# EricLBuehler/mistral.rs

Measured on AMD Instinct MI355X. Metric: decode_tokens_per_sec, higher is better.
Workload: dtype q4_k/q6_k weights x q8_k activations (int8 dot, f32 accumulate: the reference CPU path's arithmetic); 1 GPU; Llama-3-8B GGUF Q4_K_M, TP=1, 512 prefill / 1598 decode, batch 1, paged KV bf16 (block 32); parallelism=tp1

## Files before the change

### mistral.rs_amd/csrc/ext_dec.hip

```cpp
#include "dec_attn.cuh"
#include <stdio.h>
#include <stdlib.h>
#include <math.h>
#include <algorithm>
#include "../../include/mistralrs_paged_attn.h"

#include "dec_gemv.cuh"

#ifndef MRS_WAIT_VMCNT0
#define MRS_WAIT_VMCNT0() asm volatile("s_waitcnt vmcnt(0)" ::: "memory")
#endif

namespace mrs {
namespace dec {

__device__ __forceinline__ void st16(uint8_t *p, const uint8_t *b) { *(v4u *)p = *(const v4u *)b; }
__device__ __forceinline__ void k4_scale_min(const uint8_t *sc12, uint8_t *sc, uint8_t *mn) {
#pragma unroll
  for (int g = 0; g < 8; ++g) {
    if (g < 4) { sc[g] = sc12[g] & 63; mn[g] = sc12[g + 4] & 63; }
    else { sc[g] = (sc12[g + 4] & 15) | ((sc12[g - 4] >> 6) << 4); mn[g] = (sc12[g + 4] >> 4) | ((sc12[g] >> 6) << 4); }
  }
}
template <int TYPE>
__global__ void __launch_bounds__(256) repack_kernel(const uint8_t *__restrict__ src, uint8_t *__restrict__ dst, long long n, int K, long long nlanes) {
  const long long i = (long long)blockIdx.x * 256 + threadIdx.x;
  if (i >= nlanes) return;
  const Geo g = geo_for(K);
  const long long tile = i >> 6;
  const int L = (int)(i & 63), r = L >> 4, p = (L >> 2) & 3, c = L & 3, slot = L >> 2;
  const long long rg = tile / g.Cs;
  const int t = (int)(tile - rg * g.Cs);
  const long long row = rg * g.R + r;
  const int sb = p * g.Cs + t;
  const bool have = row < n && sb < g.S;
  uint8_t *tb = dst + (size_t)tile * tile_bytes(TYPE);
  alignas(16) uint8_t buf[16];
  if constexpr (TYPE == T_Q4_K || TYPE == T_Q5_K) {
    constexpr int TS = TYPE == T_Q4_K ? 144 : 176;
    constexpr unsigned HS = TYPE == T_Q4_K ? 2048u : 2560u, HD = TYPE == T_Q4_K ? 2304u : 2816u;
    const uint8_t *b = src + ((size_t)row * g.S + sb) * TS;
    const uint8_t *qs = b + (TYPE == T_Q5_K ? 48 : 16);
    for (int h = 0; h < 2; ++h) {
      for (int k = 0; k < 16; ++k) buf[k] = have ? (uint8_t)(qs[32 * c + 16 * h + k] ^ (TYPE == T_Q4_K ? 0x80 : 0x00)) : 0;
      st16(tb + (size_t)h * 1024 + (size_t)L * 16, buf);
    }
    if constexpr (TYPE == T_Q5_K) {
      const uint8_t *qh = b + 16;
      for (int h = 0; h < 2; ++h) {
        uint32_t wv = 0;
        if (have)
          for (int k = 0; k < 4; ++k)
            for (int jj = 0; jj < 4; ++jj) {
              const uint32_t v = qh[h * 16 + 4 * k + jj];
              wv |= ((v >> (2 * c)) & 1u) << (8 * jj + k);
              wv |= ((v >> (2 * c + 1)) & 1u) << (8 * jj + 4 + k);
            }
        *(uint32_t *)(tb + 2048 + (size_t)L * 8 + 4 * h) = wv;
      }
    }
    uint8_t sc[8], mn[8];
    if (have) k4_scale_min(b + 4, sc, mn);
    *(uint32_t *)(tb + HS + (size_t)L * 4) = have ? ((uint32_t)sc[2 * c] | ((uint32_t)sc[2 * c + 1] << 8) | ((uint32_t)mn[2 * c] << 16) | ((uint32_t)mn[2 * c + 1] << 24)) : 0u;
    if (c == 0) *(uint32_t *)(tb + HD + (size_t)slot * 4) = have ? ((uint32_t)b[0] | ((uint32_t)b[1] << 8) | ((uint32_t)b[2] << 16) | ((uint32_t)b[3] << 24)) : 0u;
  } else if constexpr (TYPE == T_Q6_K) {
    const uint8_t *b = src + ((size_t)row * g.S + sb) * 210;
    const uint8_t *ql = b, *qh = b + 128;
    auto lo4 = [&](int e) { const int hh = e / 128, pos = e % 32, qt = (e % 128) / 32, ii = hh * 64 + pos + (qt % 2) * 32; return qt < 2 ? (ql[ii] & 15) : (ql[ii] >> 4); };
    auto hi2 = [&](int e) { const int hh = e / 128, pos = e % 32, qt = (e % 128) / 32; return (qh[hh * 32 + pos] >> (qt * 2)) & 3; };
    for (int h = 0; h < 2; ++h) {
      for (int k = 0; k < 16; ++k) buf[k] = have ? (uint8_t)(lo4((4 * c + 2 * h) * 16 + k) | (lo4((4 * c + 2 * h + 1) * 16 + k) << 4)) : 0;
      st16(tb + (size_t)h * 1024 + (size_t)L * 16, buf);
    }
    for (int k = 0; k < 16; ++k)
      buf[k] = have ? (uint8_t)(hi2((4 * c) * 16 + k) | (hi2((4 * c + 1) * 16 + k) << 2) | (hi2((4 * c + 2) * 16 + k) << 4) | (hi2((4 * c + 3) * 16 + k) << 6)) : 0;
    st16(tb + 2048 + (size_t)L * 16, buf);
    *(uint32_t *)(tb + 3072 + (size_t)L * 4) = have ? ((uint32_t)b[192 + 4 * c] | ((uint32_t)b[193 + 4 * c] << 8) | ((uint32_t)b[194 + 4 * c] << 16) | ((uint32_t)b[195 + 4 * c] << 24)) : 0u;
    if (c == 0) *(uint16_t *)(tb + 3328 + (size_t)slot * 2) = have ? (uint16_t)(b[208] | (b[209] << 8)) : (uint16_t)0;
  } else {
    const uint8_t *b = src + ((size_t)row * (K / 32) + (size_t)sb * 8 + 2 * c) * 34;
    for (int pi = 0; pi < 4; ++pi) {
      for (int k = 0; k < 16; ++k) buf[k] = have ? b[(pi >> 1) * 34 + 2 + (pi & 1) * 16 + k] : 0;
      st16(tb + (size_t)pi * 1024 + (size_t)L * 16, buf);
    }
    *(uint32_t *)(tb + 4096 + (size_t)L * 4) = have ? ((uint32_t)b[0] | ((uint32_t)b[1] << 8) | ((uint32_t)b[34] << 16) | ((uint32_t)b[35] << 24)) : 0u;
  }
}

static bool make_mat(Mat &m, const void *planes, int type, long long n, long long k) {
  if (!planes || !dec_type(type) || n <= 0 || k <= 0 || k % 256) return false;
  const size_t tb = tensor_bytes(type, n, k);
  if (tb >= 0xF0000000ull) return false;
  m.base = (const uint8_t *)planes; m.bytes = (unsigned)tb; m.type = type; m.n = (int)n; m.k = (int)k;
  return true;
}


struct Attn2Args {
  AttnArgs t;
  unsigned *ticket;
  uint8_t *img;
};
template <int G>
__device__ __forceinline__ void attn2_merge(const Attn2Args &a, int kvh, int seq, int ns, int wave, int lane, int ncols) {
  constexpr int HD = 128, NP = (G + 1) / 2;
  const AttnArgs &t = a.t;
  if (wave >= NP) return;
  const int head0 = kvh * G, hsel = lane >> 5, head = head0 + 2 * wave + hsel;
  const bool live = 2 * wave + hsel < G;
  const size_t pA = ((size_t)seq * t.num_heads + head0 + 2 * wave) * t.max_splits;
  const size_t pB = ((size_t)seq * t.num_heads + head0 + min(2 * wave + 1, G - 1)) * t.max_splits;
  auto ldw = [&](const float *p) { return __hip_atomic_load(p, __ATOMIC_RELAXED, __HIP_MEMORY_SCOPE_AGENT); };
  const float mA = lane < ns ? ldw(t.part_m + pA + lane) : -FLT_MAX, lA = lane < ns ? ldw(t.part_l + pA + lane) : 0.f;
  const float mB = lane < ns ? ldw(t.part_m + pB + lane) : -FLT_MAX, lB = lane < ns ? ldw(t.part_l + pB + lane) : 0.f;
  const __amdgpu_buffer_rsrc_t ro = __builtin_amdgcn_make_buffer_rsrc((void *)(t.part_o + pA * HD), (short)0, (int)((pB - pA + ns) * HD * 4), 0x00020000);
  const unsigned off0 = (unsigned)(lane & 31) * 16u + (hsel ? (unsigned)((pB - pA) * HD * 4) : 0u);
  constexpr int MB = 16;
  constexpr int AUX = 16;
  v4u r[MB];
#pragma unroll
  for (int i = 0; i < MB; ++i) r[i] = __builtin_amdgcn_raw_buffer_load_b128(ro, off0 + (unsigned)i * 512u, 0, AUX);
  const float wA = fast_exp_ref(mA - dec2::wave_max_all(mA)), wB = fast_exp_ref(mB - dec2::wave_max_all(mB));
  float s_all = 0.f;
  float4 acc = make_float4(0.f, 0.f, 0.f, 0.f);
  auto step = [&](int j, v4u raw) {
    const float wAj = dec2::rlf(wA, j), wBj = dec2::rlf(wB, j), lAj = dec2::rlf(lA, j), lBj = dec2::rlf(lB, j);
    const float wj = hsel ? wBj : wAj, lj = hsel ? lBj : lAj;
    const float lw = lj * wj;
    s_all = s_all + lw;
    const float4 o = as_f4(raw);
    const float t0 = o.x * wj, t1 = o.y * wj, t2 = o.z * wj, t3 = o.w * wj;
    acc.x = acc.x + t0; acc.y = acc.y + t1; acc.z = acc.z + t2; acc.w = acc.w + t3;
  };
  for (int j0 = 0; j0 < ns; j0 += MB) {
    if (j0 > 0) {
#pragma unroll
      for (int i = 0; i < MB; ++i) r[i] = __builtin_amdgcn_raw_buffer_load_b128(ro, off0 + (unsigned)(j0 + i) * 512u, 0, AUX);
    }
#pragma unroll
    for (int i = 0; i < MB; ++i)
      if (j0 + i < ns) step(j0 + i, r[i]);
  }
  const float inv = 1.0f / s_all;
  const float4 v = make_float4(acc.x * inv, acc.y * inv, acc.z * inv, acc.w * inv);
  if (t.out && live) *(float4 *)(t.out + ((size_t)seq * t.num_heads + head) * HD + (lane & 31) * 4) = v;
  if (a.img) {
    const int K = t.num_heads * HD, sb = (head0 + 2 * wave) >> 1;
    quantize_sb(v, sb, seq, ACT_Q8K, (char *)a.img, K, ncols);
  }
}

template <int G, class CT>
__global__ void __launch_bounds__(64 * G) dec_attn2_kernel(const Attn2Args a) {
  constexpr int HD = 128;
  __shared__ __attribute__((aligned(16))) float q_s[G][HD + 32];
  __shared__ int last_s;
  const AttnArgs &t = a.t;
  const int tid = tid_opaque(), lane = tid & 63, wave = __builtin_amdgcn_readfirstlane(tid >> 6);
  const int kvh = blockIdx.x, seq = blockIdx.y;
  const int split = blockIdx.z, head0 = kvh * G;
  const unsigned blk_first = t.block_tables[(size_t)seq * t.max_blocks_per_seq + min(split * t.bpw, t.max_blocks_per_seq - 1)];
  const int nblk = ((int)t.context_lens[seq] + 31) / 32;
  const int ns = (nblk + t.bpw - 1) / t.bpw;
  if (split >= ns) return;
  {
    const int b0 = split * t.bpw, b1 = min(b0 + t.bpw, nblk);
    const int ctx_w = (int)t.context_lens[seq], lo_w = t.window > 0 && ctx_w > t.window ? ctx_w - t.window : 0;
    auto publish = [&](int, float o0, float o1, float m, float l) {
      const size_t pi = ((size_t)seq * t.num_heads + head0 + wave) * t.max_splits + split;
      __hip_atomic_store(t.part_o + pi * HD + lane, o0, __ATOMIC_RELAXED, __HIP_MEMORY_SCOPE_AGENT);
      __hip_atomic_store(t.part_o + pi * HD + lane + 64, o1, __ATOMIC_RELAXED, __HIP_MEMORY_SCOPE_AGENT);
      if (lane == 0) {
        __hip_atomic_store(t.part_m + pi, m, __ATOMIC_RELAXED, __HIP_MEMORY_SCOPE_AGENT);
        __hip_atomic_store(t.part_l + pi, l, __ATOMIC_RELAXED, __HIP_MEMORY_SCOPE_AGENT);
      }
    };
    if (b1 * 32 <= lo_w) {
      publish(0, 0.f, 0.f, -FLT_MAX, 0.f);
    } else {
      attn_split_core<1, CT>(t, kvh, head0 + wave, seq, b0, b1, q_s[wave], q_s[wave] + HD, publish, (int)blk_first);
    }
  }
  MRS_WAIT_VMCNT0();
  __syncthreads();
  unsigned *tk = a.ticket + (size_t)seq * t.num_kv_heads + kvh;
  constexpr int ticket_order = __ATOMIC_RELAXED;
  if (tid == 0) last_s = __hip_atomic_fetch_add(tk, 1u, ticket_order, __HIP_MEMORY_SCOPE_AGENT) == (unsigned)(ns - 1);
  __syncthreads();
  if (!last_s) return;
  if (tid == 0) __hip_atomic_store(tk, 0u, __ATOMIC_RELAXED, __HIP_MEMORY_SCOPE_AGENT);
  attn2_merge<G>(a, kvh, seq, ns, wave, lane, gridDim.y);
}


struct ActImgArgs {
  const float *x; int ldx; const float *norm_w; float eps; int K, mode;
  char *img;
  int gc0[8], gn[8];
};
__global__ void __launch_bounds__(NT) dec_act_image_kernel(const ActImgArgs a) {
  __shared__ float red[8];
  const int tid = tid_opaque(), wave = __builtin_amdgcn_readfirstlane(tid >> 6);
  const int c = (int)blockIdx.x;
  const float *x = a.x + (size_t)c * a.ldx;
  const ActRegs<1> pre = act_issue_all<1>(x, (unsigned)a.K * 4u, a.norm_w, a.K, wave);
  act_sumsq_all<1, 1>(red, pre, x, a.ldx, a.norm_w, a.K, wave);
  if (a.norm_w) __syncthreads();
  const int c0 = a.gc0[c], n = a.gn[c];
  act_quantize_all<1, 1>(a.img + act_bytes(a.K, c0), red, pre, x, a.ldx, a.norm_w, a.eps, a.K, a.mode, wave, c - c0, n);
}

static unsigned long long *g_tl_buf = nullptr;
template <int EPI> struct Launch {
  template <int NCOLS> static int go(GemvArgs a, hipStream_t s) {
    const Geo g = geo_for(a.K);
    constexpr int NCI = EPI == EPI_RESID2 ? 2 : NCOLS;
    a.tl = g_tl_buf;
    a.rgpu = EPI == EPI_QKV && g.R < 2 ? 2 : 1;
    const int upr = g.R * a.rgpu;
    int grid = 0;
    if (EPI == EPI_QKV) {
      double bytes[3]; double tot = 0; int want = 0;
      for (int i = 0; i < 3; ++i) {
        if (a.nrows[i] % upr) return -3;
        a.units[i] = a.nrows[i] / upr;
        bytes[i] = (double)a.units[i] * a.rgpu * g.TPC * (double)rec_bytes(a.m[i].type, g); tot += bytes[i]; want += a.units[i];
      }
      const int G = want < 256 ? want : 256;
      int wgs[3], used = 0;
      for (int i = 0; i < 3; ++i) { wgs[i] = std::max(1, std::min(a.units[i], (int)(G * bytes[i] / tot + 0.5))); used += wgs[i]; }
      while (used > G) { int big = 0; for (int i = 1; i < 3; ++i) if (wgs[i] > wgs[big]) big = i; if (wgs[big] <= 1) break; --wgs[big]; --used; }
      a.wg0[0] = 0; for (int i = 0; i < 3; ++i) a.wg0[i + 1] = a.wg0[i] + wgs[i];
      grid = a.wg0[3];
    } else {
      const int slots = a.slots > 1 ? a.slots : 1;
      if ((slots > 1 || a.expert_sel) && a.nrows[0] % upr) return -3;
      const int upe = (a.nrows[0] + upr - 1) / upr;
      a.units[0] = upe * slots;
      grid = a.units[0] < 256 ? a.units[0] : 256;
    }
    if (grid < 1) return -1;
    for (int i = 0; i < (EPI == EPI_QKV ? 3 : 1); ++i) {
      const int nwg = EPI == EPI_QKV ? a.wg0[i + 1] - a.wg0[i] : grid;
      a.ubase[i] = a.units[i] / nwg; a.urem[i] = a.units[i] % nwg;
    }
    a.upe = EPI == EPI_RESID2 ? a.units[0] : a.units[0] / (a.slots > 1 ? a.slots : 1);
    if (a.upe < 1) a.upe = 1;
    size_t lds = (act_bytes(a.K, NCI) + 15) & ~(size_t)15;
    if (lds > LDS_IMG_MAX) return -2;
    int tmask = 0;
    for (int i = 0; i < (EPI == EPI_QKV ? 3 : 1); ++i) tmask |= tmask_of(a.m[i].type);
    int total_units = 0;
    for (int i = 0; i < (EPI == EPI_QKV ? 3 : 1); ++i) total_units += a.units[i];
    static const int force_ring2 = [] { const char *e = getenv("MRS_DEC_RING2"); return e ? atoi(e) : -1; }();
    const bool ring2 = force_ring2 >= 0 ? force_ring2 != 0 : total_units >= 8 * grid;
    return gemv_launch<NCOLS>(EPI, tmask, ring2, grid, lds, a, s);
  }
  static GemvArgs shift_cols(GemvArgs a, int c0) {
    if (a.x) a.x += (size_t)c0 * a.ldx;
    if (a.out) a.out += (size_t)c0 * a.out_stride;
    if (a.qkv.q_out) a.qkv.q_out += (size_t)c0 * a.nrows[0];
    if (a.qkv.positions) a.qkv.positions += c0;
    if (a.qkv.slot_mapping) a.qkv.slot_mapping += c0;
    if (a.x_img) a.x_img = (const char *)a.x_img + act_bytes(a.K, c0);
    return a;
  }
  static int run(const GemvArgs &a, int b, hipStream_t s) {
    if (b > 1 && act_bytes(a.K, b) > LDS_IMG_MAX) {
      const int half = b / 2;
      const int rc = run(a, half, s);
      return rc ? rc : run(shift_cols(a, half), b - half, s);
    }
    switch (b) {
    case 1: return go<1>(a, s); case 2: return go<2>(a, s); case 3: return go<3>(a, s); case 4: return go<4>(a, s);
    case 5: return go<5>(a, s); case 6: return go<6>(a, s); case 7: return go<7>(a, s); case 8: return go<8>(a, s);
    default: return -1;
    }
  }
};

}
}

using namespace mrs;
using namespace mrs::dec;

struct mrs_dec_mat_c { const void *planes; int type; long long n, k; };

extern "C" void mrs_dec_timeline(void *buf, int) { g_tl_buf = (unsigned long long *)buf; }
extern "C" int mrs_dec_supported(int ggml_type) { return dec_type(ggml_type) ? 1 : 0; }
extern "C" size_t mrs_dec_repack_bytes(int type, long long n, long long k) {
  if (!dec_type(type) || k <= 0 || k % 256 || n <= 0) return 0;
  return tensor_bytes(type, n, k);
}
extern "C" int mrs_dec_repack(const void *gguf_blocks, int type, long long n, long long k, void *planes, void *stream) {
  if (!mrs_dec_repack_bytes(type, n, k) || !gguf_blocks || !planes) return -1;
  const Geo g = geo_for((int)k);
  const long long nslots = ((n + g.R - 1) / g.R) * g.TPC * 64;
  const dim3 grid((unsigned)((nslots + 255) / 256));
  hipStream_t s = (hipStream_t)stream;
  switch (type) {
  case T_Q4_K: hipLaunchKernelGGL(repack_kernel<T_Q4_K>, grid, dim3(256), 0, s, (const uint8_t *)gguf_blocks, (uint8_t *)planes, n, (int)k, nslots); break;
  case T_Q5_K: hipLaunchKernelGGL(repack_kernel<T_Q5_K>, grid, dim3(256), 0, s, (const uint8_t *)gguf_blocks, (uint8_t *)planes, n, (int)k, nslots); break;
  case T_Q6_K: hipLaunchKernelGGL(repack_kernel<T_Q6_K>, grid, dim3(256), 0, s, (const uint8_t *)gguf_blocks, (uint8_t *)planes, n, (int)k, nslots); break;
  default: hipLaunchKernelGGL(repack_kernel<T_Q8_0>, grid, dim3(256), 0, s, (const uint8_t *)gguf_blocks, (uint8_t *)planes, n, (int)k, nslots); break;
  }
  return 0;
}
static int dec_qkv_impl(const mrs_dec_mat_c *wq, const mrs_dec_mat_c *wk, const mrs_dec_mat_c *wv, const float *h, int ldh, const float *norm_w, float eps,
                        float *q_out, void *k_cache, void *v_cache, const int64_t *slot_mapping, const int32_t *positions, const float *cos_t,
                        const float *sin_t, int head_dim, int rot_pairs, int num_kv_heads, int block_size, int kv_dtype, int b, int neox, void *stream,
                        const void *x_img = nullptr) {
  GemvArgs a{};
  a.neox = neox;
  a.x_img = x_img;
  if (neox && rot_pairs * 2 != head_dim) return -1;
  if (!wq || !wk || !wv || !make_mat(a.m[0], wq->planes, wq->type, wq->n, wq->k) || !make_mat(a.m[1], wk->planes, wk->type, wk->n, wk->k) ||
      !make_mat(a.m[2], wv->planes, wv->type, wv->n, wv->k)) return -1;
  if (wq->k != wk->k || wq->k != wv->k) return -1;
  if (act_mode_for(wq->type) != act_mode_for(wk->type) || act_mode_for(wq->type) != act_mode_for(wv->type)) return -1;
  if (!qkv_epi_fill(a.qkv, q_out, k_cache, v_cache, slot_mapping, positions, cos_t, sin_t, head_dim, rot_pairs, num_kv_heads, block_size, kv_dtype, wq->n, wk->n, wv->n))
    return -1;
  a.nrows[0] = (int)wq->n; a.nrows[1] = (int)wk->n; a.nrows[2] = (int)wv->n; a.K = (int)wq->k;
  a.x = h; a.ldx = ldh; a.norm_w = norm_w; a.eps = eps;
  return Launch<EPI_QKV>::run(a, b, (hipStream_t)stream);
}
extern "C" int mrs_dec_qkv(const mrs_dec_mat_c *wq, const mrs_dec_mat_c *wk, const mrs_dec_mat_c *wv, const float *h, int ldh, const float *norm_w, float eps,
                           float *q_out, void *k_cache, void *v_cache, const int64_t *slot_mapping, const int32_t *positions, const float *cos_t,
                           const float *sin_t, int head_dim, int rot_pairs, int num_kv_heads, int block_size, int kv_dtype, int b, void *stream) {
  return dec_qkv_impl(wq, wk, wv, h, ldh, norm_w, eps, q_out, k_cache, v_cache, slot_mapping, positions, cos_t, sin_t, head_dim, rot_pairs, num_kv_heads, block_size,
                      kv_dtype, b, 0, stream);
}
extern "C" int mrs_dec_qkv_neox(const mrs_dec_mat_c *wq, const mrs_dec_mat_c *wk, const mrs_dec_mat_c *wv, const float *h, int ldh, const float *norm_w, float eps,
                                float *q_out, void *k_cache, void *v_cache, const int64_t *slot_mapping, const int32_t *positions, const float *cos_t,
                                const float *sin_t, int head_dim, int rot_pairs, int num_kv_heads, int block_size, int kv_dtype, int b, void *stream) {
  return dec_qkv_impl(wq, wk, wv, h, ldh, norm_w, eps, q_out, k_cache, v_cache, slot_mapping, positions, cos_t, sin_t, head_dim, rot_pairs, num_kv_heads, block_size,
                      kv_dtype, b, 1, stream);
}

extern "C" int mrs_dec_gate_up(const mrs_dec_mat_c *wg, const mrs_dec_mat_c *wu, int n, const int32_t *expert_sel, const float *h, int ldh, const float *norm_w,
                               float eps, int activation, float *act_out, int ld_out, int b, void *stream) {
  GemvArgs a{};
  if (!wg || !wu || !make_mat(a.m[0], wg->planes, wg->type, wg->n, wg->k) || !make_mat(a.m[1], wu->planes, wu->type, wu->n, wu->k)) return -1;
  if (wg->type != wu->type || wg->n != wu->n || wg->k != wu->k || n <= 0 || wg->n % n || (!expert_sel && wg->n != n) || wg->n / n > 256) return -1;
  a.nrows[0] = a.nrows[1] = n; a.K = (int)wg->k; a.x = h; a.ldx = ldh; a.norm_w = norm_w; a.eps = eps; a.activation = activation;
  a.out = act_out; a.out_stride = ld_out; a.expert_sel = expert_sel;
  return Launch<EPI_GLU>::run(a, b, (hipStream_t)stream);
}

extern "C" int mrs_dec_gate_up_topk(const mrs_dec_mat_c *wg, const mrs_dec_mat_c *wu, int n, const int32_t *expert_sel, int topk, const float *h, const float *norm_w,
                                    float eps, int activation, float *act_out, int ld_out, void *stream) {
  GemvArgs a{};
  if (!wg || !wu || !expert_sel || topk < 1 || topk > 8 || !make_mat(a.m[0], wg->planes, wg->type, wg->n, wg->k) || !make_mat(a.m[1], wu->planes, wu->type, wu->n, wu->k)) return -1;
  if (wg->type != wu->type || wg->n != wu->n || wg->k != wu->k || n <= 0 || wg->n % n || wg->n / n > 256) return -1;
  a.nrows[0] = a.nrows[1] = n; a.K = (int)wg->k; a.x = h; a.ldx = (int)wg->k; a.norm_w = norm_w; a.eps = eps; a.activation = activation;
  a.out = act_out; a.out_stride = ld_out; a.expert_sel = expert_sel; a.slots = topk; a.slot_out_stride = ld_out;
  return Launch<EPI_GLU>::run(a, 1, (hipStream_t)stream);
}

extern "C" int mrs_dec_proj_top2(const mrs_dec_mat_c *w, int n, const int32_t *expert_sel, const float *x, int ldx, float *out, float resid_scale,
                                 const float *acc_scale, void *stream) {
  GemvArgs a{};
  if (!w || !expert_sel || !acc_scale || !make_mat(a.m[0], w->planes, w->type, w->n, w->k) || n <= 0 || w->n % n || w->n / n > 256) return -1;
  a.nrows[0] = n; a.K = (int)w->k; a.x = x; a.ldx = ldx; a.out = out; a.out_stride = n; a.resid_scale = resid_scale; a.acc_scale = acc_scale;
  a.expert_sel = expert_sel;
  return Launch<EPI_RESID2>::go<1>(a, (hipStream_t)stream);
}

extern "C" int mrs_dec_proj(const mrs_dec_mat_c *w, int n, const int32_t *expert_sel, const float *x, int ldx, const float *norm_w, float eps, float *out,
                            int ld_out, int mode, float resid_scale, const float *acc_scale, int b, void *stream) {
  GemvArgs a{};
  if (!w || !make_mat(a.m[0], w->planes, w->type, w->n, w->k) || n <= 0 || w->n % n || (!expert_sel && w->n != n) || w->n / n > 256) return -1;
  a.nrows[0] = n; a.K = (int)w->k; a.x = x; a.ldx = ldx; a.norm_w = norm_w; a.eps = eps; a.out = out; a.out_stride = ld_out;
  a.resid_scale = resid_scale; a.acc_scale = acc_scale; a.expert_sel = expert_sel;
  return mode ? Launch<EPI_RESID>::run(a, b, (hipStream_t)stream) : Launch<EPI_STORE>::run(a, b, (hipStream_t)stream);
}

extern "C" int mrs_dec_proj_argmax(const mrs_dec_mat_c *w, int n, const float *x, int ldx, const float *norm_w, float eps, float *out, int ld_out, void *amax, void *stream) {
  GemvArgs a{};
  if (!w || !amax || !make_mat(a.m[0], w->planes, w->type, w->n, w->k) || n <= 0 || w->n != n) return -1;
  a.nrows[0] = n; a.K = (int)w->k; a.x = x; a.ldx = ldx; a.norm_w = norm_w; a.eps = eps; a.out = out; a.out_stride = ld_out; a.resid_scale = 1.0f;
  a.amax = (unsigned long long *)amax;
  return Launch<EPI_STORE>::run(a, 1, (hipStream_t)stream);
}

extern "C" int mrs_dec_proj_img(const mrs_dec_mat_c *w, int n, const void *x_img, float *out, int ld_out, int mode, float resid_scale, int b, void *stream) {
  GemvArgs a{};
  if (!w || !x_img || !make_mat(a.m[0], w->planes, w->type, w->n, w->k) || n <= 0 || w->n != n) return -1;
  a.nrows[0] = n; a.K = (int)w->k; a.x_img = x_img; a.out = out; a.out_stride = ld_out; a.resid_scale = resid_scale;
  return mode ? Launch<EPI_RESID>::run(a, b, (hipStream_t)stream) : Launch<EPI_STORE>::run(a, b, (hipStream_t)stream);
}
extern "C" size_t mrs_dec_act_image_bytes(int k, int b) { return act_bytes(k, b); }
extern "C" size_t mrs_dec_proj_img_max_bytes(void) { return LDS_IMG_MAX; }

extern "C" int mrs_dec_act_image(const float *x, int ldx, const float *norm_w, float eps, int k, int weight_type, int b, void *img_out, void *stream) {
  if (!x || !img_out || b < 1 || b > 8 || k <= 0 || k % 256 || !dec_type(weight_type) || ((uintptr_t)img_out & 15)) return -1;
  ActImgArgs a{};
  a.x = x; a.ldx = ldx; a.norm_w = norm_w; a.eps = eps; a.K = k; a.mode = act_mode_for(weight_type); a.img = (char *)img_out;
  col_groups(k, 0, b, a.gc0, a.gn);
  hipLaunchKernelGGL(dec_act_image_kernel, dim3(b), dim3(NT), 0, (hipStream_t)stream, a);
  return hipGetLastError() == hipSuccess ? 0 : -4;
}
extern "C" int mrs_dec_qkv_img(const mrs_dec_mat_c *wq, const mrs_dec_mat_c *wk, const mrs_dec_mat_c *wv, const void *x_img, float *q_out, void *k_cache, void *v_cache,
                               const int64_t *slot_mapping, const int32_t *positions, const float *cos_t, const float *sin_t, int head_dim, int rot_pairs,
                               int num_kv_heads, int block_size, int kv_dtype, int b, int neox, void *stream) {
  if (!x_img) return -1;
  return dec_qkv_impl(wq, wk, wv, nullptr, 0, nullptr, 0.f, q_out, k_cache, v_cache, slot_mapping, positions, cos_t, sin_t, head_dim, rot_pairs, num_kv_heads, block_size,
                      kv_dtype, b, neox, stream, x_img);
}
extern "C" int mrs_dec_gate_up_img(const mrs_dec_mat_c *wg, const mrs_dec_mat_c *wu, int n, const void *x_img, int activation, float *act_out, int ld_out, int b,
                                   void *stream) {
  GemvArgs a{};
  if (!x_img || !wg || !wu || !make_mat(a.m[0], wg->planes, wg->type, wg->n, wg->k) || !make_mat(a.m[1], wu->planes, wu->type, wu->n, wu->k)) return -1;
  if (wg->type != wu->type || wg->n != wu->n || wg->k != wu->k || n <= 0 || wg->n != n) return -1;
  a.nrows[0] = a.nrows[1] = n; a.K = (int)wg->k; a.x_img = x_img; a.activation = activation; a.out = act_out; a.out_stride = ld_out;
  return Launch<EPI_GLU>::run(a, b, (hipStream_t)stream);
}

extern "C" int mrs_dec_attention(float *out_f32, void *img_out, unsigned *ticket, float *part_o, float *part_m, float *part_l, const float *q, const void *k_cache,
                                 const void *v_cache, int num_kv_heads, float scale, const uint32_t *block_tables, const uint32_t *context_lens, int block_size,
                                 int max_context_len, int num_seqs, int num_heads, int head_size, int max_blocks_per_seq, int q_stride, int kv_block_stride,
                                 int kv_head_stride, int kv_dtype, int sliding_window, void *stream) {
  if (!ticket || !part_o || !part_m || !part_l || block_size != 32 || head_size != 128 || num_seqs <= 0 || num_kv_heads <= 0 || num_heads % num_kv_heads ||
      (kv_dtype != 0 && kv_dtype != 1) || max_context_len <= 0) return -1;
  const int G = num_heads / num_kv_heads;
  if (G != 1 && G != 2 && G != 4 && G != 8) return -1;
  const bool with_img = img_out && (G % 2 == 0) && num_seqs <= 8;
  if (!with_img && !out_f32) return -1;
  Attn2Args a{};
  AttnArgs &t = a.t;
  t.q = q; t.k_cache = (const uint16_t *)k_cache; t.v_cache = (const uint16_t *)v_cache; t.block_tables = block_tables; t.context_lens = context_lens;
  t.part_o = part_o; t.part_m = part_m; t.part_l = part_l; t.out = out_f32;
  t.num_heads = num_heads; t.num_kv_heads = num_kv_heads; t.max_blocks_per_seq = max_blocks_per_seq; t.q_stride = q_stride;
  t.kv_block_stride = kv_block_stride; t.kv_head_stride = kv_head_stride; t.num_seqs = num_seqs; t.scale = scale;
  t.window = sliding_window > 0 ? sliding_window : 0;
  const int nblk = (max_context_len + 31) / 32;
  t.bpw = nblk <= 64 ? 1 : (nblk + 63) / 64;
  t.max_splits = mrs_decode_attention_max_splits(max_context_len);
  a.ticket = ticket; a.img = with_img ? (uint8_t *)img_out : nullptr;
  const int nsplit = (nblk + t.bpw - 1) / t.bpw;
  const dim3 grid(num_kv_heads, num_seqs, nsplit);
  hipStream_t s = (hipStream_t)stream;
#define MRS_A2(GG, CT) hipLaunchKernelGGL((dec_attn2_kernel<GG, CT>), grid, dim3(64 * GG), 0, s, a)
#define MRS_A2G(CT) switch (G) { case 1: MRS_A2(1, CT); break; case 2: MRS_A2(2, CT); break; case 4: MRS_A2(4, CT); break; default: MRS_A2(8, CT); break; }
  if (kv_dtype == 1) { MRS_A2G(bf16_t) } else { MRS_A2G(f16_t) }
#undef MRS_A2G
#undef MRS_A2
  return with_img ? 1 : 0;
}


extern "C" size_t mrs_dec2_repack_bytes(int type, long long n, long long k) { return mrs_dec_repack_bytes(type, n, k); }
extern "C" int mrs_dec2_repack(const void *gguf_blocks, int type, long long n, long long k, void *planes, void *stream) { return mrs_dec_repack(gguf_blocks, type, n, k, planes, stream); }
extern "C" void mrs_dec2_timeline(void *buf) { g_tl_buf = (unsigned long long *)buf; }
extern "C" int mrs_dec2_gemv(const mrs_dec_mat_c *w, const float *x, int ldx, const float *norm_w, float eps, float *out, int ld_out, int b, void *stream) {
  if (!w) return -1;
  return mrs_dec_proj(w, (int)w->n, nullptr, x, ldx, norm_w, eps, out, ld_out, 0, 1.0f, nullptr, b, stream);
}
```

Before: 534.9 tokens/s.

## Pack two attention splits per block and stage merge partials in LDS

The split-KV decode attention kernel now processes two splits per workgroup (S=2), which halves the grid along the split axis and the number of ticket increments. When the last block does the merge, the otherwise idle waves prefetch the partial outputs for splits 16..31 into dynamic LDS. The merging waves then read those partials from LDS rather than issuing serial global loads. This adds dynamic shared-memory sizing, extra __syncthreads, and more template instantiations, and it may lower occupancy because blocks are larger.

```diff
diff --git a/mistral.rs_amd/csrc/ext_dec.hip b/mistral.rs_amd/csrc/ext_dec.hip
--- a/mistral.rs_amd/csrc/ext_dec.hip
+++ b/mistral.rs_amd/csrc/ext_dec.hip
@@ -100,46 +100,88 @@
   AttnArgs t;
   unsigned *ticket;
   uint8_t *img;
+  int lds_ns;
 };
-template <int G>
-__device__ __forceinline__ void attn2_merge(const Attn2Args &a, int kvh, int seq, int ns, int wave, int lane, int ncols) {
-  constexpr int HD = 128, NP = (G + 1) / 2;
+template <int G, int S>
+__device__ __forceinline__ void attn2_merge(const Attn2Args &a, int kvh, int seq, int ns, int wave, int lane, int ncols, float *lds) {
+  constexpr int HD = 128, NP = (G + 1) / 2, NH = G * S - NP;
+  constexpr int AUX = 16;
   const AttnArgs &t = a.t;
-  if (wave >= NP) return;
+  const bool staged = NH > 0 && ns > 16 && ns <= a.lds_ns;
   const int head0 = kvh * G, hsel = lane >> 5, head = head0 + 2 * wave + hsel;
   const bool live = 2 * wave + hsel < G;
-  const size_t pA = ((size_t)seq * t.num_heads + head0 + 2 * wave) * t.max_splits;
-  const size_t pB = ((size_t)seq * t.num_heads + head0 + min(2 * wave + 1, G - 1)) * t.max_splits;
+  const int hA = min(2 * wave, G - 1), hB = min(2 * wave + 1, G - 1);
+  const size_t pA = ((size_t)seq * t.num_heads + head0 + hA) * t.max_splits;
+  const size_t pB = ((size_t)seq * t.num_heads + head0 + hB) * t.max_splits;
   auto ldw = [&](const float *p) { return __hip_atomic_load(p, __ATOMIC_RELAXED, __HIP_MEMORY_SCOPE_AGENT); };
-  const float mA = lane < ns ? ldw(t.part_m + pA + lane) : -FLT_MAX, lA = lane < ns ? ldw(t.part_l + pA + lane) : 0.f;
-  const float mB = lane < ns ? ldw(t.part_m + pB + lane) : -FLT_MAX, lB = lane < ns ? ldw(t.part_l + pB + lane) : 0.f;
-  const __amdgpu_buffer_rsrc_t ro = __builtin_amdgcn_make_buffer_rsrc((void *)(t.part_o + pA * HD), (short)0, (int)((pB - pA + ns) * HD * 4), 0x00020000);
-  const unsigned off0 = (unsigned)(lane & 31) * 16u + (hsel ? (unsigned)((pB - pA) * HD * 4) : 0u);
-  constexpr int MB = 16;
-  constexpr int AUX = 16;
-  v4u r[MB];
-#pragma unroll
-  for (int i = 0; i < MB; ++i) r[i] = __builtin_amdgcn_raw_buffer_load_b128(ro, off0 + (unsigned)i * 512u, 0, AUX);
-  const float wA = fast_exp_ref(mA - dec2::wave_max_all(mA)), wB = fast_exp_ref(mB - dec2::wave_max_all(mB));
+  const bool ml = wave < NP && lane < ns;
+  const float mA = ml ? ldw(t.part_m + pA + lane) : -FLT_MAX, lA = ml ? ldw(t.part_l + pA + lane) : 0.f;
+  const float mB = ml ? ldw(t.part_m + pB + lane) : -FLT_MAX, lB = ml ? ldw(t.part_l + pB + lane) : 0.f;
   float s_all = 0.f;
   float4 acc = make_float4(0.f, 0.f, 0.f, 0.f);
-  auto step = [&](int j, v4u raw) {
+  float wA, wB;
+  auto step = [&](int j, float4 o) {
     const float wAj = dec2::rlf(wA, j), wBj = dec2::rlf(wB, j), lAj = dec2::rlf(lA, j), lBj = dec2::rlf(lB, j);
     const float wj = hsel ? wBj : wAj, lj = hsel ? lBj : lAj;
     const float lw = lj * wj;
     s_all = s_all + lw;
-    const float4 o = as_f4(raw);
     const float t0 = o.x * wj, t1 = o.y * wj, t2 = o.z * wj, t3 = o.w * wj;
     acc.x = acc.x + t0; acc.y = acc.y + t1; acc.z = acc.z + t2; acc.w = acc.w + t3;
   };
-  for (int j0 = 0; j0 < ns; j0 += MB) {
-    if (j0 > 0) {
-#pragma unroll
-      for (int i = 0; i < MB; ++i) r[i] = __builtin_amdgcn_raw_buffer_load_b128(ro, off0 + (unsigned)(j0 + i) * 512u, 0, AUX);
-    }
+  if (wave >= NP) {
+    if constexpr (NH > 0) {
+      if (!staged) return;
+      constexpr int NU = (8 * G + NH - 1) / NH;
+      const int hw = wave - NP;
+      const size_t p0 = ((size_t)seq * t.num_heads + head0) * t.max_splits;
+      const __amdgpu_buffer_rsrc_t rh = __builtin_amdgcn_make_buffer_rsrc((void *)(t.part_o + p0 * HD), (short)0, (int)(((size_t)(G - 1) * t.max_splits + ns) * HD * 4), 0x00020000);
+      v4u r[NU];
+#pragma unroll
+      for (int i = 0; i < NU; ++i) {
+        const int u = hw + i * NH, g = u % G, j = 16 + 2 * (u / G) + hsel;
+        r[i] = __builtin_amdgcn_raw_buffer_load_b128(rh, u < 8 * G && j < ns ? (unsigned)(g * t.max_splits + j) * 512u + (unsigned)(lane & 31) * 16u : 0xFFFFFFF0u, 0, AUX);
+      }
+#pragma unroll
+      for (int i = 0; i < NU; ++i) {
+        const int u = hw + i * NH, g = u % G, j = 16 + 2 * (u / G) + hsel;
+        if (u < 8 * G && j < ns) *(v4u *)(lds + ((size_t)g * 16 + (j - 16)) * HD + (lane & 31) * 4) = r[i];
+      }
+      __syncthreads();
+    }
+    return;
+  }
+  {
+    const __amdgpu_buffer_rsrc_t ro = __builtin_amdgcn_make_buffer_rsrc((void *)(t.part_o + pA * HD), (short)0, (int)((pB - pA + ns) * HD * 4), 0x00020000);
+    const unsigned off0 = (unsigned)(lane & 31) * 16u + (hsel ? (unsigned)((pB - pA) * HD * 4) : 0u);
+    constexpr int MB = 16;
+    v4u r[MB];
+#pragma unroll
+    for (int i = 0; i < MB; ++i) r[i] = __builtin_amdgcn_raw_buffer_load_b128(ro, off0 + (unsigned)i * 512u, 0, AUX);
+    wA = fast_exp_ref(mA - dec2::wave_max_all(mA)), wB = fast_exp_ref(mB - dec2::wave_max_all(mB));
 #pragma unroll
     for (int i = 0; i < MB; ++i)
-      if (j0 + i < ns) step(j0 + i, r[i]);
+      if (i < ns) step(i, as_f4(r[i]));
+    if (staged) {
+      __syncthreads();
+      const float *lo = lds + (size_t)(hsel ? hB : hA) * 16 * HD + (lane & 31) * 4;
+      constexpr int RB = 8;
+      for (int j0 = 16; j0 < ns; j0 += RB) {
+        float4 o[RB];
+#pragma unroll
+        for (int i = 0; i < RB; ++i) o[i] = *(const float4 *)(lo + (size_t)(min(j0 + i, ns - 1) - 16) * HD);
+#pragma unroll
+        for (int i = 0; i < RB; ++i)
+          if (j0 + i < ns) step(j0 + i, o[i]);
+      }
+    } else {
+      for (int j0 = MB; j0 < ns; j0 += MB) {
+#pragma unroll
+        for (int i = 0; i < MB; ++i) r[i] = __builtin_amdgcn_raw_buffer_load_b128(ro, off0 + (unsigned)(j0 + i) * 512u, 0, AUX);
+#pragma unroll
+        for (int i = 0; i < MB; ++i)
+          if (j0 + i < ns) step(j0 + i, as_f4(r[i]));
+      }
+    }
   }
   const float inv = 1.0f / s_all;
   const float4 v = make_float4(acc.x * inv, acc.y * inv, acc.z * inv, acc.w * inv);
@@ -150,24 +192,26 @@
   }
 }
 
-template <int G, class CT>
-__global__ void __launch_bounds__(64 * G) dec_attn2_kernel(const Attn2Args a) {
+template <int G, int S, class CT>
+__global__ void __launch_bounds__(64 * G * S) dec_attn2_kernel(const Attn2Args a) {
   constexpr int HD = 128;
-  __shared__ __attribute__((aligned(16))) float q_s[G][HD + 32];
+  extern __shared__ __attribute__((aligned(16))) char smem[];
+  float *lds = (float *)smem;
   __shared__ int last_s;
   const AttnArgs &t = a.t;
   const int tid = tid_opaque(), lane = tid & 63, wave = __builtin_amdgcn_readfirstlane(tid >> 6);
   const int kvh = blockIdx.x, seq = blockIdx.y;
-  const int split = blockIdx.z, head0 = kvh * G;
+  const int split = (int)blockIdx.z * S + wave / G, head0 = kvh * G, g = wave % G;
   const unsigned blk_first = t.block_tables[(size_t)seq * t.max_blocks_per_seq + min(split * t.bpw, t.max_blocks_per_seq - 1)];
   const int nblk = ((int)t.context_lens[seq] + 31) / 32;
   const int ns = (nblk + t.bpw - 1) / t.bpw;
-  if (split >= ns) return;
-  {
+  if ((int)blockIdx.z * S >= ns) return;
+  if (split < ns) {
+    float *q_s = lds + wave * (HD + 32);
     const int b0 = split * t.bpw, b1 = min(b0 + t.bpw, nblk);
     const int ctx_w = (int)t.context_lens[seq], lo_w = t.window > 0 && ctx_w > t.window ? ctx_w - t.window : 0;
     auto publish = [&](int, float o0, float o1, float m, float l) {
-      const size_t pi = ((size_t)seq * t.num_heads + head0 + wave) * t.max_splits + split;
+      const size_t pi = ((size_t)seq * t.num_heads + head0 + g) * t.max_splits + split;
       __hip_atomic_store(t.part_o + pi * HD + lane, o0, __ATOMIC_RELAXED, __HIP_MEMORY_SCOPE_AGENT);
       __hip_atomic_store(t.part_o + pi * HD + lane + 64, o1, __ATOMIC_RELAXED, __HIP_MEMORY_SCOPE_AGENT);
       if (lane == 0) {
@@ -178,18 +222,18 @@
     if (b1 * 32 <= lo_w) {
       publish(0, 0.f, 0.f, -FLT_MAX, 0.f);
     } else {
-      attn_split_core<1, CT>(t, kvh, head0 + wave, seq, b0, b1, q_s[wave], q_s[wave] + HD, publish, (int)blk_first);
+      attn_split_core<1, CT>(t, kvh, head0 + g, seq, b0, b1, q_s, q_s + HD, publish, (int)blk_first);
     }
   }
   MRS_WAIT_VMCNT0();
   __syncthreads();
   unsigned *tk = a.ticket + (size_t)seq * t.num_kv_heads + kvh;
   constexpr int ticket_order = __ATOMIC_RELAXED;
-  if (tid == 0) last_s = __hip_atomic_fetch_add(tk, 1u, ticket_order, __HIP_MEMORY_SCOPE_AGENT) == (unsigned)(ns - 1);
+  if (tid == 0) last_s = __hip_atomic_fetch_add(tk, 1u, ticket_order, __HIP_MEMORY_SCOPE_AGENT) == (unsigned)((ns + S - 1) / S - 1);
   __syncthreads();
   if (!last_s) return;
   if (tid == 0) __hip_atomic_store(tk, 0u, __ATOMIC_RELAXED, __HIP_MEMORY_SCOPE_AGENT);
-  attn2_merge<G>(a, kvh, seq, ns, wave, lane, gridDim.y);
+  attn2_merge<G, S>(a, kvh, seq, ns, wave, lane, gridDim.y, lds);
 }
 
 
@@ -439,12 +483,18 @@
   t.max_splits = mrs_decode_attention_max_splits(max_context_len);
   a.ticket = ticket; a.img = with_img ? (uint8_t *)img_out : nullptr;
   const int nsplit = (nblk + t.bpw - 1) / t.bpw;
-  const dim3 grid(num_kv_heads, num_seqs, nsplit);
+  const int S = nsplit >= 2 ? 2 : 1;
+  a.lds_ns = nsplit > 16 && nsplit <= 32 ? 32 : 0;
+  const int lds_bytes = std::max(G * S * (128 + 32) * 4, a.lds_ns ? G * 16 * 128 * 4 : 0);
+  const dim3 grid(num_kv_heads, num_seqs, (nsplit + S - 1) / S);
   hipStream_t s = (hipStream_t)stream;
-#define MRS_A2(GG, CT) hipLaunchKernelGGL((dec_attn2_kernel<GG, CT>), grid, dim3(64 * GG), 0, s, a)
-#define MRS_A2G(CT) switch (G) { case 1: MRS_A2(1, CT); break; case 2: MRS_A2(2, CT); break; case 4: MRS_A2(4, CT); break; default: MRS_A2(8, CT); break; }
+#define MRS_A2(GG, SS, CT) do { lds_attr_once((const void *)dec_attn2_kernel<GG, SS, CT>, LDS_DYN_MAX); \
+    hipLaunchKernelGGL((dec_attn2_kernel<GG, SS, CT>), grid, dim3(64 * GG * SS), lds_bytes, s, a); } while (0)
+#define MRS_A2S(GG, CT) if (S == 1) MRS_A2(GG, 1, CT); else MRS_A2(GG, 2, CT)
+#define MRS_A2G(CT) switch (G) { case 1: MRS_A2S(1, CT); break; case 2: MRS_A2S(2, CT); break; case 4: MRS_A2S(4, CT); break; default: MRS_A2S(8, CT); break; }
   if (kv_dtype == 1) { MRS_A2G(bf16_t) } else { MRS_A2G(f16_t) }
 #undef MRS_A2G
+#undef MRS_A2S
 #undef MRS_A2
   return with_img ? 1 : 0;
 }
```

Result: no change. 534.4 tokens/s, median of 2 (-0.1%).
